# LeonhardFeiner/sparse_rcnn

Measured on AMD Instinct MI355X. Metric: active-voxels/sec fwd+bwd, ScanNet U-Net backbone, higher is better.
Workload: dtype f32

## Files before the change

sparse_rcnn_amd/csrc/scn_common.h:

```cpp
#pragma once
#include <hip/hip_runtime.h>
#include <atomic>
#include <stdint.h>
#include <stdio.h>
#include <string.h>

#include "../../include/scn_mi355x.h"

namespace scn {

extern thread_local char g_err[512];

inline int fail(int code, const char* fmt, const char* a = "", long long b = 0, long long c = 0) {
    snprintf(g_err, sizeof(g_err), fmt, a, b, c);
    return code;
}

#define SCN_HIP(expr)                                                                               \
    do {                                                                                            \
        hipError_t e_ = (expr);                                                                     \
        if (e_ != hipSuccess) {                                                                     \
            snprintf(scn::g_err, sizeof(scn::g_err), "%s failed: %s (%s:%d)", #expr,                \
                     hipGetErrorString(e_), __FILE__, __LINE__);                                    \
            return SCN_EHIP;                                                                        \
        }                                                                                           \
    } while (0)

#define SCN_LAUNCH_CHECK()                                                                          \
    do {                                                                                            \
        hipError_t e_ = hipGetLastError();                                                          \
        if (e_ != hipSuccess) {                                                                     \
            snprintf(scn::g_err, sizeof(scn::g_err), "kernel launch failed: %s (%s:%d)",            \
                     hipGetErrorString(e_), __FILE__, __LINE__);                                    \
            return SCN_EHIP;                                                                        \
        }                                                                                           \
    } while (0)

#define SCN_REQUIRE(cond)                                                                           \
    do {                                                                                            \
        if (!(cond)) {                                                                              \
            snprintf(scn::g_err, sizeof(scn::g_err), "%s: requirement failed: %s", __func__, #cond); \
            return SCN_EINVAL;                                                                      \
        }                                                                                           \
    } while (0)

enum Switch {
    SW_TS_SPLIT, SW_TS_SPLIT_MAX, SW_TS_NO_TAIL, SW_TS_W_HALF, SW_TS_W_BOTH, SW_TB_NB, SW_TB_KH, SW_TB_STREAM,
    SW_TB_NO_XORDER, SW_TS_STREAM, SW_TSS_NW, SW_EXEC_DEFER_SUMS, SW_PYRAMID_V1, SW_PYRAMID_ONE_STREAM, SW_WD_NO_T3,
    SW_WGRAD_BF16_MFMA, SW_WGRAD_SPLITS, SW_WD_NO_EVEC, SW_PYRAMID_NO_BRICKS, SW_CU_BUDGET, SW_EXP_A, SW_EXP_B, SW_TS_NO_CHAIN, SW_TS_PROG, SW_TB_NO_BINS,
    SW_EXEC_GROUP_WGRAD, SW_EXEC_GROUP_STEP, SW_COUNT
};
struct SwitchVal { bool set = false; long long i = 0; double f = 0.0; };
SwitchVal sw(Switch s);
inline int cu_budget() { const SwitchVal v = sw(SW_CU_BUDGET); return (v.set && v.i >= 32 && v.i <= 256) ? (int)v.i : 256; }

struct DeviceOnce {
    std::atomic<uint64_t> mask{0};
    static int cur() { int d = 0; return (hipGetDevice(&d) == hipSuccess && d >= 0 && d < 64) ? d : -1; }
    bool needed() const { const int d = cur(); return d < 0 || !(mask.load(std::memory_order_acquire) & (1ull << d)); }
    void done() { const int d = cur(); if (d >= 0) mask.fetch_or(1ull << d, std::memory_order_release); }
};

int wgrad_defer_group(bool on);

inline hipStream_t S(scn_stream_t s) { return reinterpret_cast<hipStream_t>(s); }

inline int64_t cdiv(int64_t a, int64_t b) { return (a + b - 1) / b; }

inline int ew_grid(int64_t work_items, int block) {
    int64_t g = cdiv(work_items, block);
    if (g > 256 * 8) g = 256 * 8;
    if (g < 1) g = 1;
    return (int)g;
}

int add_relu(const float* X, const float* X1, int64_t count, float* Y, scn_stream_t stream);
int add_relu_bf16(const uint16_t* X, const uint16_t* X1, int64_t count, uint16_t* Y, scn_stream_t stream);

}

#define SCN_EMPTY_KEY 0xFFFFFFFFFFFFFFFFull

__device__ __forceinline__ unsigned long long scn_pack_key(int x, int y, int z, int b) {
    return ((unsigned long long)(unsigned)b << 48) | ((unsigned long long)(unsigned)x << 32) |
           ((unsigned long long)(unsigned)y << 16) | (unsigned long long)(unsigned)z;
}

__device__ __forceinline__ unsigned long long scn_hash_slot(unsigned long long key, unsigned long long mask) {
    unsigned long long h = key;
    h ^= h >> 33;
    h *= 0xff51afd7ed558ccdull;
    h ^= h >> 33;
    h *= 0xc4ceb9fe1a85ec53ull;
    h ^= h >> 33;
    return h & mask;
}

__device__ __forceinline__ float scn_mask_sigmoid(float x) { return 1.f / (1.f + __expf(-x)); }

__device__ __forceinline__ float scn_box_iou(const float* as, const float* ae, float area_a, const float* bx) {
#pragma clang fp contract(off)
    float inter = 1.f;
#pragma unroll
    for (int d = 0; d < 3; ++d) {
        const float lo = fmaxf(as[d], bx[d]), hi = fminf(ae[d], bx[3 + d]);
        const float e = fmaxf((hi - lo), 0.f);
        inter = d == 0 ? e : (inter * e);
    }
    const float uni = (area_a + bx[6]) - inter;
    return (inter / uni);
}
```

sparse_rcnn_amd/csrc/scn_conv.hip:

```cpp
#include "scn_common.h"

using scn::S;
using scn::cdiv;

namespace scn {
bool gemm_lt_usable(const void* X0, const void* X1, int cx0, int cx1, const void* W);
int gemm_lt_rows(const void* X0, int cx0, const void* X1, int cx1, int64_t n, const float* W, const float* bias,
                 const void* residual, const void* relu_mask, void* Y0, int cy0, void* Y1, int cy1, int flags, bool hb,
                 scn_stream_t stream);
int gemm_lt_rules(const void* X, int cin, const int32_t* in_rows, const int32_t* out_rows, const int64_t* prefix_host,
                  int n_off, const float* W, const float* bias, const void* relu_mask, void* Y, int cout, int flags,
                  bool hb, scn_stream_t stream);
}

typedef float f32x16 __attribute__((ext_vector_type(16)));

#define MFMA(a, b, c) __builtin_amdgcn_mfma_f32_32x32x2f32((a), (b), (c), 0, 0, 0)

__device__ __forceinline__ int acc_row(int v, int h) { return (v & 3) + 8 * (v >> 2) + 4 * h; }

__device__ __forceinline__ float bf16_bits_to_f32(unsigned short h) { return __uint_as_float((unsigned)h << 16); }
__device__ __forceinline__ unsigned short f32_to_bf16_bits(float f) { return __builtin_bit_cast(unsigned short, (__bf16)f); }

template <bool FAST, bool WT, bool HB = false>
__device__ __forceinline__ void tile_mac(f32x16& acc, const float* __restrict__ xrow, bool have, int cin,
                                         const float* __restrict__ Wo, int cout, int n, bool n_ok, int h, bool relu_in) {
    const unsigned short* xh = (const unsigned short*)xrow;
    if (FAST) {
        for (int q = 0; q < cin; q += 8) {
            const int k0 = q + 4 * h;
            float4 a = make_float4(0.f, 0.f, 0.f, 0.f);
            if (HB) {
                if (have) {
                    const uint2 r = *(const uint2*)(xh + k0);
                    a = make_float4(__uint_as_float(r.x << 16), __uint_as_float(r.x & 0xffff0000u),
                                    __uint_as_float(r.y << 16), __uint_as_float(r.y & 0xffff0000u));
                }
            } else if (have) a = *(const float4*)(xrow + k0);
            if (relu_in) { a.x = fmaxf(a.x, 0.f); a.y = fmaxf(a.y, 0.f); a.z = fmaxf(a.z, 0.f); a.w = fmaxf(a.w, 0.f); }
            float4 b;
            if (WT) {
                b = n_ok ? *(const float4*)(Wo + (long long)n * cin + k0) : make_float4(0.f, 0.f, 0.f, 0.f);
            } else {
                const float* wp = Wo + (long long)k0 * cout + n;
                b.x = n_ok ? wp[0] : 0.f;
                b.y = n_ok ? wp[cout] : 0.f;
                b.z = n_ok ? wp[2 * cout] : 0.f;
                b.w = n_ok ? wp[3 * cout] : 0.f;
            }
            acc = MFMA(a.x, b.x, acc);
            acc = MFMA(a.y, b.y, acc);
            acc = MFMA(a.z, b.z, acc);
            acc = MFMA(a.w, b.w, acc);
        }
    } else {
        for (int q = 0; q < cin; q += 8) {
#pragma unroll
            for (int e = 0; e < 4; ++e) {
                const int k = q + 4 * h + e;
                const bool k_ok = k < cin;
                float a = (have && k_ok) ? (HB ? bf16_bits_to_f32(xh[k]) : xrow[k]) : 0.f;
                if (relu_in) a = fmaxf(a, 0.f);
                float b = 0.f;
                if (k_ok && n_ok) b = WT ? Wo[(long long)n * cin + k] : Wo[(long long)k * cout + n];
                acc = MFMA(a, b, acc);
            }
        }
    }
}

template <bool FAST, bool WT, bool HB = false>
__global__ __launch_bounds__(256) void k_gemm_table(const float* __restrict__ X, int cin,
                                                    const int* __restrict__ table, int n_off, long long n_out,
                                                    const float* __restrict__ W, const float* __restrict__ bias,
                                                    const float* __restrict__ residual,
                                                    const float* __restrict__ relu_mask, float* __restrict__ Y, int cout,
                                                    int flags) {
    const int lane = threadIdx.x & 63, wave = threadIdx.x >> 6;
    const int m = lane & 31, h = lane >> 5;
    const long long r0 = ((long long)blockIdx.x * 4 + wave) * 32;
    if (r0 >= n_out) return;
    const long long row = r0 + m;
    const bool row_ok = row < n_out;
    const int n0 = blockIdx.y * 32;
    const int n = n0 + m;
    const bool n_ok = n < cout;
    const bool relu_in = flags & SCN_F_RELU_IN;
    const bool rev = flags & SCN_F_OFF_REVERSE;
    const long long wstride = (long long)cin * cout;

    f32x16 acc;
#pragma unroll
    for (int v = 0; v < 16; ++v) acc[v] = 0.f;

    int idx_next = row_ok ? (table ? table[row] : (int)row) : -1;
    for (int o = 0; o < n_off; ++o) {
        const int idx = idx_next;
        if (o + 1 < n_off) idx_next = row_ok ? table[(long long)(o + 1) * n_out + row] : -1;
        if (__ballot(idx >= 0) == 0ull) continue;
        const float* Wo = W + (long long)(rev ? n_off - 1 - o : o) * wstride;
        const float* xrow = HB ? (const float*)((const unsigned short*)X + (long long)(idx >= 0 ? idx : 0) * cin)
                               : X + (long long)(idx >= 0 ? idx : 0) * cin;
        tile_mac<FAST, WT, HB>(acc, xrow, idx >= 0, cin, Wo, cout, n, n_ok, h, relu_in);
    }

    const float bv = (bias && n_ok) ? bias[n] : 0.f;
#pragma unroll
    for (int v = 0; v < 16; ++v) {
        const long long r = r0 + acc_row(v, h);
        if (r < n_out && n_ok) {
            const long long off = r * cout + n;
            float y = acc[v] + bv;
            if (HB) {
                if (residual) y += bf16_bits_to_f32(((const unsigned short*)residual)[off]);
                if (relu_mask && !(bf16_bits_to_f32(((const unsigned short*)relu_mask)[off]) > 0.f)) y = 0.f;
                ((unsigned short*)Y)[off] = f32_to_bf16_bits(y);
            } else {
                if (residual) y += residual[off];
                if (relu_mask && !(relu_mask[off] > 0.f)) y = 0.f;
                Y[off] = y;
            }
        }
    }
}

static int gemm_table_impl(const float* X, int64_t n_in, int cin, const int32_t* table, int n_off, int64_t n_out,
                           const float* W, const float* bias, const float* residual, const float* relu_mask,
                           float* Y, int cout, int flags, scn_stream_t stream, bool hb) {
    SCN_REQUIRE(n_in >= 0 && n_out >= 0 && cin >= 1 && cout >= 1 && n_off >= 1);
    SCN_REQUIRE(table || (n_off == 1 && n_in == n_out));
    if (n_out == 0) return SCN_OK;
    SCN_REQUIRE(X && W && Y);
    SCN_REQUIRE(n_out * (int64_t)cout < (1LL << 40) && cdiv(n_out, 128) < 2147483647LL);
    const bool fast = (cin % 8 == 0) && (((uintptr_t)X & 15) == 0) && (((uintptr_t)W & 15) == 0);
    const bool wt = flags & SCN_F_W_TRANSPOSED;
    if (!table && fast && !(flags & SCN_F_GEMM_V1) && n_out < 2147483647LL)
        return scn::gemm_lt_rows(X, cin, nullptr, 0, n_out, W, bias, residual, relu_mask, Y, cout, nullptr, 0, flags, hb,
                                 stream);
    dim3 grid((unsigned)cdiv(n_out, 128), (unsigned)cdiv(cout, 32));
#define LAUNCH_T(F, T, H)                                                                                     \
    hipLaunchKernelGGL((k_gemm_table<F, T, H>), grid, dim3(256), 0, S(stream), X, cin, table, n_off,          \
                       (long long)n_out, W, bias, residual, relu_mask, Y, cout, flags)
#define PICK_T(H)                                                                                             \
    do {                                                                                                      \
        if (fast && wt) LAUNCH_T(true, true, H);                                                              \
        else if (fast) LAUNCH_T(true, false, H);                                                              \
        else if (wt) LAUNCH_T(false, true, H);                                                                \
        else LAUNCH_T(false, false, H);                                                                       \
    } while (0)
    if (hb) PICK_T(true); else PICK_T(false);
#undef PICK_T
#undef LAUNCH_T
    SCN_LAUNCH_CHECK();
    return SCN_OK;
}

extern "C" int scn_gemm_table(const float* X, int64_t n_in, int cin, const int32_t* table, int n_off, int64_t n_out,
                              const float* W, const float* bias, const float* residual, const float* relu_mask,
                              float* Y, int cout, int flags, scn_stream_t stream) {
    return gemm_table_impl(X, n_in, cin, table, n_off, n_out, W, bias, residual, relu_mask, Y, cout, flags, stream, false);
}

extern "C" int scn_gemm_table_bf16(const uint16_t* X, int64_t n_in, int cin, const int32_t* table, int n_off,
                                   int64_t n_out, const float* W, const float* bias, const uint16_t* residual,
                                   const uint16_t* relu_mask, uint16_t* Y, int cout, int flags, scn_stream_t stream) {
    return gemm_table_impl((const float*)X, n_in, cin, table, n_off, n_out, W, bias, (const float*)residual,
                           (const float*)relu_mask, (float*)Y, cout, flags, stream, true);
}

struct SegTiles {
    long long rule_start[33];
    long long tile_start[33];
    int n_off;
};

template <bool FAST, bool WT, bool HB = false>
__global__ __launch_bounds__(256) void k_gemm_rules(const float* __restrict__ X, int cin,
                                                    const int* __restrict__ in_rows, const int* __restrict__ out_rows,
                                                    SegTiles seg, const float* __restrict__ W,
                                                    const float* __restrict__ bias, const float* __restrict__ relu_mask,
                                                    float* __restrict__ Y, int cout, int flags) {
    const int lane = threadIdx.x & 63, wave = threadIdx.x >> 6;
    const int m = lane & 31, h = lane >> 5;
    const long long tile = (long long)blockIdx.x * 4 + wave;
    if (tile >= seg.tile_start[seg.n_off]) return;
    int o = 0;
    while (tile >= seg.tile_start[o + 1]) ++o;
    const long long p0 = seg.rule_start[o] + (tile - seg.tile_start[o]) * 32;
    const long long p_end = seg.rule_start[o + 1];
    const long long p = p0 + m;
    const bool p_ok = p < p_end;
    const int idx = p_ok ? in_rows[p] : -1;
    const int orow = p_ok ? out_rows[p] : -1;
    const int n0 = blockIdx.y * 32;
    const int n = n0 + m;
    const bool n_ok = n < cout;

    f32x16 acc;
#pragma unroll
    for (int v = 0; v < 16; ++v) acc[v] = 0.f;
    const float* Wo = W + (long long)o * cin * cout;
    const float* xrow = HB ? (const float*)((const unsigned short*)X + (long long)(idx >= 0 ? idx : 0) * cin)
                           : X + (long long)(idx >= 0 ? idx : 0) * cin;
    tile_mac<FAST, WT, HB>(acc, xrow, idx >= 0, cin, Wo, cout, n, n_ok, h, flags & SCN_F_RELU_IN);

    const float bv = (bias && n_ok) ? bias[n] : 0.f;
#pragma unroll
    for (int v = 0; v < 16; ++v) {
        const int r = __shfl(orow, acc_row(v, h));
        if (r >= 0 && n_ok) {
            const long long off = (long long)r * cout + n;
            float y = acc[v] + bv;
            if (HB) {
                if (relu_mask && !(bf16_bits_to_f32(((const unsigned short*)relu_mask)[off]) > 0.f)) y = 0.f;
                ((unsigned short*)Y)[off] = f32_to_bf16_bits(y);
            } else {
                if (relu_mask && !(relu_mask[off] > 0.f)) y = 0.f;
                Y[off] = y;
            }
        }
    }
}

static int make_seg_tiles(const int64_t* prefix_host, int n_off, int tile, SegTiles& seg) {
    seg.n_off = n_off;
    seg.rule_start[0] = prefix_host[0];
    seg.tile_start[0] = 0;
    for (int o = 0; o < n_off; ++o) {
        int64_t cnt = prefix_host[o + 1] - prefix_host[o];
        if (cnt < 0) return SCN_EINVAL;
        seg.rule_start[o + 1] = prefix_host[o + 1];
        seg.tile_start[o + 1] = seg.tile_start[o] + cdiv(cnt, tile);
    }
    return SCN_OK;
}

static int gemm_rules_impl(const float* X, int cin, const int32_t* in_rows, const int32_t* out_rows,
                           const int64_t* prefix_host, int n_off, const float* W, const float* bias,
                           const float* relu_mask, float* Y, int cout, int flags, scn_stream_t stream, bool hb) {
    SCN_REQUIRE(prefix_host && n_off >= 1 && n_off <= 32 && cin >= 1 && cout >= 1);
    SegTiles seg;
    SCN_REQUIRE(make_seg_tiles(prefix_host, n_off, 32, seg) == SCN_OK);
    const long long tiles = seg.tile_start[n_off];
    if (tiles == 0) return SCN_OK;
    SCN_REQUIRE(X && in_rows && out_rows && W && Y);
    const bool fast = (cin % 8 == 0) && (((uintptr_t)X & 15) == 0) && (((uintptr_t)W & 15) == 0);
    const bool wt = flags & SCN_F_W_TRANSPOSED;
    if (fast && cout > 32 && !(flags & SCN_F_GEMM_V1))
        return scn::gemm_lt_rules(X, cin, in_rows, out_rows, prefix_host, n_off, W, bias, relu_mask, Y, cout, flags, hb,
                                  stream);
    dim3 grid((unsigned)cdiv(tiles, 4), (unsigned)cdiv(cout, 32));
#define LAUNCH_R(F, T, H)                                                                                     \
    hipLaunchKernelGGL((k_gemm_rules<F, T, H>), grid, dim3(256), 0, S(stream), X, cin, in_rows, out_rows, seg, \
                       W, bias, relu_mask, Y, cout, flags)
#define PICK_R(H)                                                                                             \
    do {                                                                                                      \
        if (fast && wt) LAUNCH_R(true, true, H);                                                              \
        else if (fast) LAUNCH_R(true, false, H);                                                              \
        else if (wt) LAUNCH_R(false, true, H);                                                                \
        else LAUNCH_R(false, false, H);                                                                       \
    } while (0)
    if (hb) PICK_R(true); else PICK_R(false);
#undef PICK_R
#undef LAUNCH_R
    SCN_LAUNCH_CHECK();
    return SCN_OK;
}

extern "C" int scn_gemm_rules(const float* X, int cin, const int32_t* in_rows, const int32_t* out_rows,
                              const int64_t* prefix_host, int n_off, const float* W, const float* bias,
                              const float* relu_mask, float* Y, int cout, int flags, scn_stream_t stream) {
    return gemm_rules_impl(X, cin, in_rows, out_rows, prefix_host, n_off, W, bias, relu_mask, Y, cout, flags, stream,
                           false);
}

extern "C" int scn_gemm_rules_bf16(const uint16_t* X, int cin, const int32_t* in_rows, const int32_t* out_rows,
                                   const int64_t* prefix_host, int n_off, const float* W, const float* bias,
                                   const uint16_t* relu_mask, uint16_t* Y, int cout, int flags, scn_stream_t stream) {
    return gemm_rules_impl((const float*)X, cin, in_rows, out_rows, prefix_host, n_off, W, bias,
                           (const float*)relu_mask, (float*)Y, cout, flags, stream, true);
}

template <bool HB>
__global__ __launch_bounds__(256) void k_colsum_partial(const float* __restrict__ dY, long long n, int c,
                                                        float* __restrict__ partial) {
    const unsigned short* dYh = (const unsigned short*)dY;
    const long long rows_per_block = (n + gridDim.x - 1) / gridDim.x;
    const long long r_lo = blockIdx.x * rows_per_block;
    long long r_hi = r_lo + rows_per_block;
    if (r_hi > n) r_hi = n;
    __shared__ float red[256];
    for (int c0 = 0; c0 < c; c0 += 256) {
        const int width = min(256, c - c0);
        const int lanes_per_row = width;
        const int rows_par = 256 / lanes_per_row > 0 ? 256 / lanes_per_row : 1;
        const int col = threadIdx.x % lanes_per_row;
        const int rsub = threadIdx.x / lanes_per_row;
        float s = 0.f;
        if (rsub < rows_par)
            for (long long r = r_lo + rsub; r < r_hi; r += rows_par)
                s += HB ? bf16_bits_to_f32(dYh[r * c + c0 + col]) : dY[r * c + c0 + col];
        red[threadIdx.x] = (rsub < rows_par) ? s : 0.f;
        __syncthreads();
        if (threadIdx.x < width) {
            float t = 0.f;
            for (int k = 0; k < rows_par; ++k) t += red[k * lanes_per_row + threadIdx.x];
            partial[(long long)blockIdx.x * c + c0 + threadIdx.x] = t;
        }
        __syncthreads();
    }
}

__global__ __launch_bounds__(256) void k_colsum_final(const float* __restrict__ partial, int nblk, int c,
                                                      float* __restrict__ db) {
    const int col = blockIdx.x;
    float s = 0.f;
    for (int b = threadIdx.x; b < nblk; b += 256) s += partial[(long long)b * c + col];
#pragma unroll
    for (int d = 32; d >= 1; d >>= 1) s += __shfl_down(s, d);
    __shared__ float w[4];
    if ((threadIdx.x & 63) == 0) w[threadIdx.x >> 6] = s;
    __syncthreads();
    if (threadIdx.x == 0) db[col] = (w[0] + w[1]) + (w[2] + w[3]);
}

static int colsum_impl(const float* dY, int64_t n, int c, float* db, void* scratch, scn_stream_t stream, bool hb) {
    SCN_REQUIRE(n >= 0 && c >= 1 && db && scratch);
    int nblk = (int)(n < SCN_COLSUM_BLOCKS * 8 ? cdiv(n, 8) : SCN_COLSUM_BLOCKS);
    if (nblk < 1) nblk = 1;
    if (n > 0) SCN_REQUIRE(dY);
    if (hb)
        hipLaunchKernelGGL(k_colsum_partial<true>, dim3(nblk), dim3(256), 0, S(stream), dY, (long long)n, c, (float*)scratch);
    else
        hipLaunchKernelGGL(k_colsum_partial<false>, dim3(nblk), dim3(256), 0, S(stream), dY, (long long)n, c, (float*)scratch);
    SCN_LAUNCH_CHECK();
    hipLaunchKernelGGL(k_colsum_final, dim3(c), dim3(256), 0, S(stream), (const float*)scratch, nblk, c, db);
    SCN_LAUNCH_CHECK();
    return SCN_OK;
}

extern "C" int scn_colsum(const float* dY, int64_t n, int c, float* db, void* scratch, scn_stream_t stream) {
    return colsum_impl(dY, n, c, db, scratch, stream, false);
}

extern "C" int scn_colsum_bf16(const uint16_t* dY, int64_t n, int c, float* db, void* scratch, scn_stream_t stream) {
    return colsum_impl((const float*)dY, n, c, db, scratch, stream, true);
}
```

sparse_rcnn_amd/csrc/scn_debug.hip:

```cpp
#include <stdlib.h>

#include <mutex>

#include "scn_common.h"

namespace scn {
namespace {
struct Entry { const char* name; SwitchVal v; };
Entry g_sw[SW_COUNT] = {
    {"SCN_TS_SPLIT", {}},        {"SCN_TS_SPLIT_MAX", {}},  {"SCN_TS_NO_TAIL", {}},       {"SCN_TS_W_HALF", {}},
    {"SCN_TS_W_BOTH", {}},       {"SCN_TB_NB", {}},         {"SCN_TB_KH", {}},            {"SCN_TB_STREAM", {}},
    {"SCN_TB_NO_XORDER", {}},    {"SCN_TS_STREAM", {}},     {"SCN_TSS_NW", {}},           {"SCN_EXEC_DEFER_SUMS", {}},
    {"SCN_PYRAMID_V1", {}},      {"SCN_PYRAMID_ONE_STREAM", {}}, {"SCN_WD_NO_T3", {}},    {"SCN_WGRAD_BF16_MFMA", {}},
    {"SCN_WGRAD_SPLITS", {}},    {"SCN_WD_NO_EVEC", {}},    {"SCN_PYRAMID_NO_BRICKS", {}},            {"SCN_CU_BUDGET", {}},
    {"SCN_EXP_A", {}},           {"SCN_EXP_B", {}},         {"SCN_TS_NO_CHAIN", {}},
    {"SCN_TS_PROG", {}},         {"SCN_TB_NO_BINS", {}},    {"SCN_EXEC_GROUP_WGRAD", {}},
    {"SCN_EXEC_GROUP_STEP", {}},
};
std::once_flag g_once;
std::mutex g_mu;

void assign(SwitchVal& v, const char* s) {
    v.set = s != nullptr;
    v.i = s ? atoll(s) : 0;
    v.f = s ? atof(s) : 0.0;
}
void load_env() {
    for (int k = 0; k < SW_COUNT; ++k) assign(g_sw[k].v, getenv(g_sw[k].name));
}
}

SwitchVal sw(Switch s) {
    std::call_once(g_once, load_env);
    std::lock_guard<std::mutex> lock(g_mu);
    return g_sw[s].v;
}
}

extern "C" int scn_debug_set(const char* name, const char* value) {
    SCN_REQUIRE(name != nullptr);
    std::call_once(scn::g_once, scn::load_env);
    std::lock_guard<std::mutex> lock(scn::g_mu);
    for (int k = 0; k < scn::SW_COUNT; ++k)
        if (strcmp(scn::g_sw[k].name, name) == 0) {
            scn::assign(scn::g_sw[k].v, value);
            return SCN_OK;
        }
    return scn::fail(SCN_EINVAL, "scn_debug_set: no switch named %s", name);
}

extern "C" int scn_debug_get(const char* name, int* is_set, int64_t* value) {
    SCN_REQUIRE(name != nullptr);
    for (int k = 0; k < scn::SW_COUNT; ++k)
        if (strcmp(scn::g_sw[k].name, name) == 0) {
            const scn::SwitchVal v = scn::sw((scn::Switch)k);
            if (is_set) *is_set = v.set ? 1 : 0;
            if (value) *value = v.i;
            return SCN_OK;
        }
    return scn::fail(SCN_EINVAL, "scn_debug_get: no switch named %s", name);
}
```

sparse_rcnn_amd/csrc/scn_gemm_lt.hip:

```cpp
#include "scn_common.h"

using scn::S;
using scn::cdiv;

typedef float f32x16 __attribute__((ext_vector_type(16)));
#define MFMA32(a, b, c) __builtin_amdgcn_mfma_f32_32x32x2f32((a), (b), (c), 0, 0, 0)

namespace {

constexpr int KC = 32;
constexpr int PITCH = KC + 4;

struct LtSeg {
    long long rule_start[33];
    long long tile_start[33];
    int n_off;
};

struct LtArgs {
    const void* X0; const void* X1; int cx0, cx1;
    void* Y0; void* Y1; int cy0, cy1;
    const float* W; const float* bias; const void* residual; const void* relu_mask;
    const int* in_rows; const int* out_rows;
    long long n;
    int cin, cout, flags;
};

__device__ __forceinline__ float bf16w(unsigned short h) { return __uint_as_float((unsigned)h << 16); }
__device__ __forceinline__ unsigned short bf16n(float f) { return __builtin_bit_cast(unsigned short, (__bf16)f); }
__device__ __forceinline__ int acc_row(int v, int h) { return (v & 3) + 8 * (v >> 2) + 4 * h; }

template <int NC, bool WT, bool HB, bool RULES>
__global__ __launch_bounds__(256) void k_gemm_lt(LtArgs a, LtSeg seg) {
    constexpr int RT = 128 / NC;
    constexpr int NP = RT / 32;
    __shared__ float As[2][RT * PITCH];
    const int tid = threadIdx.x, lane = tid & 63, wave = tid >> 6;
    const int m = lane & 31, h = lane >> 5;
    const int rsub = wave / NC, cchunk = wave % NC;

    long long p0, p_end;
    const float* Wo = a.W;
    if (RULES) {
        const long long tile = blockIdx.x;
        int o = 0;
        while (tile >= seg.tile_start[o + 1]) ++o;
        p0 = seg.rule_start[o] + (tile - seg.tile_start[o]) * RT;
        p_end = seg.rule_start[o + 1];
        Wo += (long long)o * a.cin * a.cout;
    } else {
        p0 = (long long)blockIdx.x * RT;
        p_end = a.n;
    }
    const int n = blockIdx.y * (NC * 32) + cchunk * 32 + m;
    const bool n_ok = n < a.cout;
    const bool relu_in = a.flags & SCN_F_RELU_IN;

    int srow[NP];
#pragma unroll
    for (int i = 0; i < NP; ++i) {
        const long long p = p0 + (tid + 256 * i) / 8;
        srow[i] = -1;
        if (p < p_end) srow[i] = RULES ? a.in_rows[p] : (int)p;
    }
    const int c4 = 4 * (tid & 7);

    auto load_a = [&](int kc, float4 (&st)[NP]) {
        const int k = kc + c4;
        const bool second = a.cx1 && k >= a.cx0;
        const char* base = (const char*)(second ? a.X1 : a.X0);
        const int pitch = second ? a.cx1 : a.cx0, kk = second ? k - a.cx0 : k;
#pragma unroll
        for (int i = 0; i < NP; ++i) {
            float4 v = make_float4(0.f, 0.f, 0.f, 0.f);
            if (srow[i] >= 0 && k < a.cin) {
                if (HB) {
                    const uint2 r = *(const uint2*)(base + 2 * ((long long)srow[i] * pitch + kk));
                    v = make_float4(__uint_as_float(r.x << 16), __uint_as_float(r.x & 0xffff0000u),
                                    __uint_as_float(r.y << 16), __uint_as_float(r.y & 0xffff0000u));
                } else {
                    v = *(const float4*)(base + 4 * ((long long)srow[i] * pitch + kk));
                }
                if (relu_in) { v.x = fmaxf(v.x, 0.f); v.y = fmaxf(v.y, 0.f); v.z = fmaxf(v.z, 0.f); v.w = fmaxf(v.w, 0.f); }
            }
            st[i] = v;
        }
    };
    auto park_a = [&](int buf, const float4 (&st)[NP]) {
#pragma unroll
        for (int i = 0; i < NP; ++i) *(float4*)&As[buf][((tid + 256 * i) / 8) * PITCH + c4] = st[i];
    };
    auto load_b = [&](int kc, float4 (&b)[4]) {
#pragma unroll
        for (int q = 0; q < 4; ++q) {
            const int k0 = kc + 8 * q + 4 * h;
            float4 v = make_float4(0.f, 0.f, 0.f, 0.f);
            if (n_ok && k0 < a.cin) {
                if (WT) {
                    v = *(const float4*)(Wo + (long long)n * a.cin + k0);
                } else {
                    const float* wp = Wo + (long long)k0 * a.cout + n;
                    v = make_float4(wp[0], wp[a.cout], wp[2 * a.cout], wp[3 * a.cout]);
                }
            }
            b[q] = v;
        }
    };

    f32x16 acc;
#pragma unroll
    for (int v = 0; v < 16; ++v) acc[v] = 0.f;

    float4 st[NP], bcur[4], bnext[4];
    load_a(0, st);
    load_b(0, bcur);
    park_a(0, st);
    __syncthreads();
    const int n_chunks = (a.cin + KC - 1) / KC;
    for (int c = 0; c < n_chunks; ++c) {
        const int buf = c & 1;
        const bool more = c + 1 < n_chunks;
        if (more) {
            load_a((c + 1) * KC, st);
            load_b((c + 1) * KC, bnext);
        }
        const float* arow = &As[buf][(rsub * 32 + m) * PITCH + 4 * h];
#pragma unroll
        for (int q = 0; q < 4; ++q) {
            const float4 av = *(const float4*)(arow + 8 * q);
            acc = MFMA32(av.x, bcur[q].x, acc);
            acc = MFMA32(av.y, bcur[q].y, acc);
            acc = MFMA32(av.z, bcur[q].z, acc);
            acc = MFMA32(av.w, bcur[q].w, acc);
        }
        if (more) {
            park_a(buf ^ 1, st);
#pragma unroll
            for (int q = 0; q < 4; ++q) bcur[q] = bnext[q];
        }
        __syncthreads();
    }

    const long long prow = p0 + rsub * 32 + m;
    long long orow_l = -1;
    if (prow < p_end) orow_l = RULES ? (long long)a.out_rows[prow] : prow;
    const int orow_i = (int)orow_l;
    const float bv = (a.bias && n_ok) ? a.bias[n] : 0.f;
    const bool second = a.cy1 && n >= a.cy0;
    char* ybase = (char*)(second ? a.Y1 : a.Y0);
    const int ypitch = second ? a.cy1 : a.cy0, yn = second ? n - a.cy0 : n;
#pragma unroll
    for (int v = 0; v < 16; ++v) {
        const int r = __shfl(orow_i, acc_row(v, h));
        if (r >= 0 && n_ok) {
            const long long off = (long long)r * ypitch + yn;
            float y = acc[v] + bv;
            if (HB) {
                if (a.residual) y += bf16w(((const unsigned short*)a.residual)[off]);
                if (a.relu_mask && !(bf16w(((const unsigned short*)a.relu_mask)[off]) > 0.f)) y = 0.f;
                ((unsigned short*)ybase)[off] = bf16n(y);
            } else {
                if (a.residual) y += ((const float*)a.residual)[off];
                if (a.relu_mask && !(((const float*)a.relu_mask)[off] > 0.f)) y = 0.f;
                ((float*)ybase)[off] = y;
            }
        }
    }
}

template <bool WT, bool HB, bool RULES>
int launch_nc(const LtArgs& a, const LtSeg& seg, long long tiles_of_128, scn_stream_t stream) {
    const int nc = a.cout <= 32 ? 1 : a.cout <= 64 ? 2 : 4;
    const unsigned gy = (unsigned)cdiv(a.cout, nc * 32);
    (void)tiles_of_128;
    long long gx;
    if (RULES) gx = seg.tile_start[seg.n_off];
    else gx = cdiv(a.n, 128 / nc);
    if (gx <= 0) return SCN_OK;
    SCN_REQUIRE(gx < 2147483647LL);
    dim3 grid((unsigned)gx, gy);
    if (nc == 1) hipLaunchKernelGGL((k_gemm_lt<1, WT, HB, RULES>), grid, dim3(256), 0, S(stream), a, seg);
    else if (nc == 2) hipLaunchKernelGGL((k_gemm_lt<2, WT, HB, RULES>), grid, dim3(256), 0, S(stream), a, seg);
    else hipLaunchKernelGGL((k_gemm_lt<4, WT, HB, RULES>), grid, dim3(256), 0, S(stream), a, seg);
    SCN_LAUNCH_CHECK();
    return SCN_OK;
}

template <bool RULES>
int launch_lt(const LtArgs& a, const LtSeg& seg, bool hb, scn_stream_t stream) {
    const bool wt = a.flags & SCN_F_W_TRANSPOSED;
    if (hb) return wt ? launch_nc<true, true, RULES>(a, seg, 0, stream) : launch_nc<false, true, RULES>(a, seg, 0, stream);
    return wt ? launch_nc<true, false, RULES>(a, seg, 0, stream) : launch_nc<false, false, RULES>(a, seg, 0, stream);
}

}

namespace scn {

bool gemm_lt_usable(const void* X0, const void* X1, int cx0, int cx1, const void* W) {
    auto al = [](const void* p) { return ((uintptr_t)p & 15) == 0; };
    return cx0 % 8 == 0 && cx1 % 8 == 0 && al(X0) && al(X1) && al(W);
}

int gemm_lt_rows(const void* X0, int cx0, const void* X1, int cx1, int64_t n, const float* W, const float* bias,
                 const void* residual, const void* relu_mask, void* Y0, int cy0, void* Y1, int cy1, int flags, bool hb,
                 scn_stream_t stream) {
    LtArgs a{};
    a.X0 = X0; a.X1 = X1; a.cx0 = cx0; a.cx1 = cx1;
    a.Y0 = Y0; a.Y1 = Y1; a.cy0 = cy0; a.cy1 = cy1;
    a.W = W; a.bias = bias; a.residual = residual; a.relu_mask = relu_mask;
    a.n = n; a.cin = cx0 + cx1; a.cout = cy0 + cy1; a.flags = flags;
    LtSeg seg{};
    return launch_lt<false>(a, seg, hb, stream);
}

int gemm_lt_rules(const void* X, int cin, const int32_t* in_rows, const int32_t* out_rows, const int64_t* prefix_host,
                  int n_off, const float* W, const float* bias, const void* relu_mask, void* Y, int cout, int flags,
                  bool hb, scn_stream_t stream) {
    LtArgs a{};
    a.X0 = X; a.cx0 = cin; a.Y0 = Y; a.cy0 = cout;
    a.W = W; a.bias = bias; a.relu_mask = relu_mask; a.in_rows = in_rows; a.out_rows = out_rows;
    a.cin = cin; a.cout = cout; a.flags = flags;
    const int nc = cout <= 32 ? 1 : cout <= 64 ? 2 : 4;
    const int rt = 128 / nc;
    LtSeg seg{};
    seg.n_off = n_off;
    seg.rule_start[0] = prefix_host[0];
    seg.tile_start[0] = 0;
    for (int o = 0; o < n_off; ++o) {
        const int64_t cnt = prefix_host[o + 1] - prefix_host[o];
        SCN_REQUIRE(cnt >= 0);
        seg.rule_start[o + 1] = prefix_host[o + 1];
        seg.tile_start[o + 1] = seg.tile_start[o] + cdiv(cnt, rt);
    }
    return launch_lt<true>(a, seg, hb, stream);
}

}

extern "C" int scn_gemm_rows2(const void* X0, int cx0, const void* X1, int cx1, int64_t n, const float* W,
                              const float* bias, const void* residual, const void* relu_mask, void* Y0, int cy0, void* Y1,
                              int cy1, int flags, int bf16_storage, scn_stream_t stream) {
    SCN_REQUIRE(n >= 0 && cx0 >= 8 && cx1 >= 0 && cy0 >= 1 && cy1 >= 0);
    SCN_REQUIRE(cx0 % 8 == 0 && cx1 % 8 == 0);
    SCN_REQUIRE((cx1 == 0) == (X1 == nullptr) && (cy1 == 0) == (Y1 == nullptr));
    SCN_REQUIRE(!(cx1 && cy1));
    SCN_REQUIRE(cy1 == 0 || (!residual && !relu_mask));
    SCN_REQUIRE(n < 2147483647LL);
    if (n == 0) return SCN_OK;
    SCN_REQUIRE(X0 && W && Y0);
    SCN_REQUIRE(scn::gemm_lt_usable(X0, X1, cx0, cx1, W));
    return scn::gemm_lt_rows(X0, cx0, X1, cx1, n, W, bias, residual, relu_mask, Y0, cy0, Y1, cy1, flags,
                             bf16_storage != 0, stream);
}
```

Measured before the change: 28.52 million.

## Make LT GEMM persistent with deep A prefetch and early epilogue loads

Reworks the MFMA row/rule GEMM kernel into a grid-sized launch. Blocks loop over flattened (row-tile, column-block) tiles and prefetch the next tile's rows and first chunk. For larger cin it adds a variant that keeps several K-chunks of A in flight, using unconditional clamped loads plus masks. It also issues residual/relu-mask loads before the final MAC, and uses readfirstlane scalar offsets and 32-bit addressing. The aim is to hide global-load latency and cut launch and tail cost, at the price of higher register pressure (launch_bounds 256,4), an occupancy query, and more complex control flow.

After: 28.52 million. No clear change (-0.0%).

```diff
diff --git a/sparse_rcnn_amd/csrc/scn_common.h b/sparse_rcnn_amd/csrc/scn_common.h
--- a/sparse_rcnn_amd/csrc/scn_common.h
+++ b/sparse_rcnn_amd/csrc/scn_common.h
@@ -48,7 +48,7 @@
     SW_TS_SPLIT, SW_TS_SPLIT_MAX, SW_TS_NO_TAIL, SW_TS_W_HALF, SW_TS_W_BOTH, SW_TB_NB, SW_TB_KH, SW_TB_STREAM,
     SW_TB_NO_XORDER, SW_TS_STREAM, SW_TSS_NW, SW_EXEC_DEFER_SUMS, SW_PYRAMID_V1, SW_PYRAMID_ONE_STREAM, SW_WD_NO_T3,
     SW_WGRAD_BF16_MFMA, SW_WGRAD_SPLITS, SW_WD_NO_EVEC, SW_PYRAMID_NO_BRICKS, SW_CU_BUDGET, SW_EXP_A, SW_EXP_B, SW_TS_NO_CHAIN, SW_TS_PROG, SW_TB_NO_BINS,
-    SW_EXEC_GROUP_WGRAD, SW_EXEC_GROUP_STEP, SW_COUNT
+    SW_EXEC_GROUP_WGRAD, SW_EXEC_GROUP_STEP, SW_GEMM_LT_WG, SW_COUNT
 };
 struct SwitchVal { bool set = false; long long i = 0; double f = 0.0; };
 SwitchVal sw(Switch s);
diff --git a/sparse_rcnn_amd/csrc/scn_conv.hip b/sparse_rcnn_amd/csrc/scn_conv.hip
--- a/sparse_rcnn_amd/csrc/scn_conv.hip
+++ b/sparse_rcnn_amd/csrc/scn_conv.hip
@@ -4,7 +4,7 @@
 using scn::cdiv;
 
 namespace scn {
-bool gemm_lt_usable(const void* X0, const void* X1, int cx0, int cx1, const void* W);
+bool gemm_lt_usable(const void* X0, const void* X1, int cx0, int cx1, const void* W, int cout);
 int gemm_lt_rows(const void* X0, int cx0, const void* X1, int cx1, int64_t n, const float* W, const float* bias,
                  const void* residual, const void* relu_mask, void* Y0, int cy0, void* Y1, int cy1, int flags, bool hb,
                  scn_stream_t stream);
@@ -134,7 +134,8 @@
     SCN_REQUIRE(n_out * (int64_t)cout < (1LL << 40) && cdiv(n_out, 128) < 2147483647LL);
     const bool fast = (cin % 8 == 0) && (((uintptr_t)X & 15) == 0) && (((uintptr_t)W & 15) == 0);
     const bool wt = flags & SCN_F_W_TRANSPOSED;
-    if (!table && fast && !(flags & SCN_F_GEMM_V1) && n_out < 2147483647LL)
+    if (!table && fast && scn::gemm_lt_usable(X, nullptr, cin, 0, W, cout) && !(flags & SCN_F_GEMM_V1) &&
+        n_out < 2147483647LL)
         return scn::gemm_lt_rows(X, cin, nullptr, 0, n_out, W, bias, residual, relu_mask, Y, cout, nullptr, 0, flags, hb,
                                  stream);
     dim3 grid((unsigned)cdiv(n_out, 128), (unsigned)cdiv(cout, 32));
@@ -246,7 +247,7 @@
     SCN_REQUIRE(X && in_rows && out_rows && W && Y);
     const bool fast = (cin % 8 == 0) && (((uintptr_t)X & 15) == 0) && (((uintptr_t)W & 15) == 0);
     const bool wt = flags & SCN_F_W_TRANSPOSED;
-    if (fast && cout > 32 && !(flags & SCN_F_GEMM_V1))
+    if (fast && cout > 32 && scn::gemm_lt_usable(X, nullptr, cin, 0, W, cout) && !(flags & SCN_F_GEMM_V1))
         return scn::gemm_lt_rules(X, cin, in_rows, out_rows, prefix_host, n_off, W, bias, relu_mask, Y, cout, flags, hb,
                                   stream);
     dim3 grid((unsigned)cdiv(tiles, 4), (unsigned)cdiv(cout, 32));
diff --git a/sparse_rcnn_amd/csrc/scn_debug.hip b/sparse_rcnn_amd/csrc/scn_debug.hip
--- a/sparse_rcnn_amd/csrc/scn_debug.hip
+++ b/sparse_rcnn_amd/csrc/scn_debug.hip
@@ -15,7 +15,7 @@
     {"SCN_WGRAD_SPLITS", {}},    {"SCN_WD_NO_EVEC", {}},    {"SCN_PYRAMID_NO_BRICKS", {}},            {"SCN_CU_BUDGET", {}},
     {"SCN_EXP_A", {}},           {"SCN_EXP_B", {}},         {"SCN_TS_NO_CHAIN", {}},
     {"SCN_TS_PROG", {}},         {"SCN_TB_NO_BINS", {}},    {"SCN_EXEC_GROUP_WGRAD", {}},
-    {"SCN_EXEC_GROUP_STEP", {}},
+    {"SCN_EXEC_GROUP_STEP", {}}, {"SCN_GEMM_LT_WG", {}},
 };
 std::once_flag g_once;
 std::mutex g_mu;
diff --git a/sparse_rcnn_amd/csrc/scn_gemm_lt.hip b/sparse_rcnn_amd/csrc/scn_gemm_lt.hip
--- a/sparse_rcnn_amd/csrc/scn_gemm_lt.hip
+++ b/sparse_rcnn_amd/csrc/scn_gemm_lt.hip
@@ -8,6 +8,12 @@
 
 namespace {
 
+#ifndef LT_EARLY
+#define LT_EARLY 1
+#endif
+#ifndef LT_DEEP
+#define LT_DEEP 4
+#endif
 constexpr int KC = 32;
 constexpr int PITCH = KC + 4;
 
@@ -24,182 +30,374 @@
     const int* in_rows; const int* out_rows;
     long long n;
     int cin, cout, flags;
+    long long n_tiles; int gy;
 };
 
 __device__ __forceinline__ float bf16w(unsigned short h) { return __uint_as_float((unsigned)h << 16); }
 __device__ __forceinline__ unsigned short bf16n(float f) { return __builtin_bit_cast(unsigned short, (__bf16)f); }
 __device__ __forceinline__ int acc_row(int v, int h) { return (v & 3) + 8 * (v >> 2) + 4 * h; }
 
-template <int NC, bool WT, bool HB, bool RULES>
-__global__ __launch_bounds__(256) void k_gemm_lt(LtArgs a, LtSeg seg) {
+struct LtTile {
+    long long p0, p_end;
+    const float* Wo;
+    int cb;
+};
+
+template <int NC, bool WT, bool HB, bool RULES, int AD>
+__global__ __launch_bounds__(256, 4) void k_gemm_lt(LtArgs a, LtSeg seg) {
     constexpr int RT = 128 / NC;
     constexpr int NP = RT / 32;
+    constexpr int ES = HB ? 2 : 4;
+    constexpr bool EARLY = LT_EARLY && WT && NC > 1;
     __shared__ float As[2][RT * PITCH];
-    const int tid = threadIdx.x, lane = tid & 63, wave = tid >> 6;
+    const int tid = threadIdx.x, lane = tid & 63, wave = __builtin_amdgcn_readfirstlane(tid >> 6);
     const int m = lane & 31, h = lane >> 5;
     const int rsub = wave / NC, cchunk = wave % NC;
-
-    long long p0, p_end;
-    const float* Wo = a.W;
-    if (RULES) {
-        const long long tile = blockIdx.x;
-        int o = 0;
-        while (tile >= seg.tile_start[o + 1]) ++o;
-        p0 = seg.rule_start[o] + (tile - seg.tile_start[o]) * RT;
-        p_end = seg.rule_start[o + 1];
-        Wo += (long long)o * a.cin * a.cout;
-    } else {
-        p0 = (long long)blockIdx.x * RT;
-        p_end = a.n;
-    }
-    const int n = blockIdx.y * (NC * 32) + cchunk * 32 + m;
-    const bool n_ok = n < a.cout;
     const bool relu_in = a.flags & SCN_F_RELU_IN;
-
-    int srow[NP];
-#pragma unroll
-    for (int i = 0; i < NP; ++i) {
-        const long long p = p0 + (tid + 256 * i) / 8;
-        srow[i] = -1;
-        if (p < p_end) srow[i] = RULES ? a.in_rows[p] : (int)p;
-    }
-    const int c4 = 4 * (tid & 7);
-
-    auto load_a = [&](int kc, float4 (&st)[NP]) {
+    const int c4 = 4 * (tid & 7), srl = tid >> 3;
+
+    auto tile_of = [&](long long t, int& o, LtTile& T) {
+        const long long rt = a.gy == 1 ? t : t / a.gy;
+        T.cb = (int)(t - rt * a.gy);
+        if (RULES) {
+            while (rt >= seg.tile_start[o + 1]) ++o;
+            T.p0 = seg.rule_start[o] + (rt - seg.tile_start[o]) * RT;
+            T.p_end = seg.rule_start[o + 1];
+            T.Wo = a.W + (long long)o * a.cin * a.cout;
+        } else {
+            T.p0 = rt * RT;
+            T.p_end = a.n;
+            T.Wo = a.W;
+        }
+    };
+    auto stage_rows = [&](const LtTile& T, int (&sr)[NP]) {
+        if (!RULES) return;
+#pragma unroll
+        for (int i = 0; i < NP; ++i) {
+            const long long p = T.p0 + srl + 32 * i;
+            const bool ok = p < T.p_end;
+            const int v = a.in_rows[ok ? p : T.p_end - 1];
+            sr[i] = ok ? v : -1;
+        }
+    };
+    auto out_row = [&](const LtTile& T) -> int {
+        if (!RULES) return -1;
+        const long long p = T.p0 + rsub * 32 + m;
+        const bool ok = p < T.p_end;
+        const int v = a.out_rows[ok ? p : T.p_end - 1];
+        return ok ? v : -1;
+    };
+    auto load_a = [&](const LtTile& T, const int (&sr)[NP], int kc, float4 (&st)[NP]) {
         const int k = kc + c4;
         const bool second = a.cx1 && k >= a.cx0;
         const char* base = (const char*)(second ? a.X1 : a.X0);
         const int pitch = second ? a.cx1 : a.cx0, kk = second ? k - a.cx0 : k;
+        const char* tbase = base + ES * (T.p0 * pitch);
 #pragma unroll
         for (int i = 0; i < NP; ++i) {
             float4 v = make_float4(0.f, 0.f, 0.f, 0.f);
-            if (srow[i] >= 0 && k < a.cin) {
+            const bool ok = RULES ? sr[i] >= 0 : T.p0 + srl + 32 * i < T.p_end;
+            if (ok && k < a.cin) {
+                const char* src = RULES ? base + ES * ((long long)sr[i] * pitch + kk)
+                                        : tbase + (unsigned)(ES * ((srl + 32 * i) * pitch + kk));
                 if (HB) {
-                    const uint2 r = *(const uint2*)(base + 2 * ((long long)srow[i] * pitch + kk));
+                    const uint2 r = *(const uint2*)src;
                     v = make_float4(__uint_as_float(r.x << 16), __uint_as_float(r.x & 0xffff0000u),
                                     __uint_as_float(r.y << 16), __uint_as_float(r.y & 0xffff0000u));
                 } else {
-                    v = *(const float4*)(base + 4 * ((long long)srow[i] * pitch + kk));
+                    v = *(const float4*)src;
                 }
-                if (relu_in) { v.x = fmaxf(v.x, 0.f); v.y = fmaxf(v.y, 0.f); v.z = fmaxf(v.z, 0.f); v.w = fmaxf(v.w, 0.f); }
             }
             st[i] = v;
         }
     };
-    auto park_a = [&](int buf, const float4 (&st)[NP]) {
-#pragma unroll
-        for (int i = 0; i < NP; ++i) *(float4*)&As[buf][((tid + 256 * i) / 8) * PITCH + c4] = st[i];
-    };
-    auto load_b = [&](int kc, float4 (&b)[4]) {
+    auto park_a = [&](int buf, const float4 (&st)[NP], int okm) {
+#pragma unroll
+        for (int i = 0; i < NP; ++i) {
+            float4 v = st[i];
+            if (!((okm >> i) & 1)) v = make_float4(0.f, 0.f, 0.f, 0.f);
+            if (relu_in) { v.x = fmaxf(v.x, 0.f); v.y = fmaxf(v.y, 0.f); v.z = fmaxf(v.z, 0.f); v.w = fmaxf(v.w, 0.f); }
+            *(float4*)&As[buf][(srl + 32 * i) * PITCH + c4] = v;
+        }
+    };
+    auto load_b = [&](const LtTile& T, int kc, float4 (&b)[4]) {
+        const int n = T.cb * (NC * 32) + cchunk * 32 + m;
 #pragma unroll
         for (int q = 0; q < 4; ++q) {
             const int k0 = kc + 8 * q + 4 * h;
             float4 v = make_float4(0.f, 0.f, 0.f, 0.f);
-            if (n_ok && k0 < a.cin) {
+            if (n < a.cout && k0 < a.cin) {
                 if (WT) {
-                    v = *(const float4*)(Wo + (long long)n * a.cin + k0);
+                    v = *(const float4*)(T.Wo + (unsigned)(n * a.cin + k0));
                 } else {
-                    const float* wp = Wo + (long long)k0 * a.cout + n;
-                    v = make_float4(wp[0], wp[a.cout], wp[2 * a.cout], wp[3 * a.cout]);
+                    const unsigned wl = (unsigned)(4 * h * a.cout + n);
+                    float e[4];
+#pragma unroll
+                    for (int j = 0; j < 4; ++j) {
+                        const unsigned ws = __builtin_amdgcn_readfirstlane((unsigned)((kc + 8 * q + j) * a.cout));
+                        e[j] = T.Wo[ws + wl];
+                    }
+                    v = make_float4(e[0], e[1], e[2], e[3]);
                 }
             }
             b[q] = v;
         }
     };
 
-    f32x16 acc;
-#pragma unroll
-    for (int v = 0; v < 16; ++v) acc[v] = 0.f;
-
-    float4 st[NP], bcur[4], bnext[4];
-    load_a(0, st);
-    load_b(0, bcur);
-    park_a(0, st);
+    auto load_a_u = [&](const LtTile& T, const int (&sr)[NP], int kc, float4 (&st)[NP], int& okm) {
+        okm = 0;
+        const int k = kc + c4, kq = k < a.cin ? k : a.cin - 4;
+        const bool second = a.cx1 && kq >= a.cx0;
+        const char* base = (const char*)(second ? a.X1 : a.X0);
+        const int pitch = second ? a.cx1 : a.cx0, kk = second ? kq - a.cx0 : kq;
+        const char* tbase = base + ES * (T.p0 * pitch);
+        const int last_row = (int)(T.p_end - 1 - T.p0 < RT - 1 ? T.p_end - 1 - T.p0 : RT - 1);
+#pragma unroll
+        for (int i = 0; i < NP; ++i) {
+            const int lr = srl + 32 * i;
+            const bool ok = (RULES ? sr[i] >= 0 : lr <= last_row) && k < a.cin;
+            const char* src = RULES ? base + ES * ((long long)(sr[i] > 0 ? sr[i] : 0) * pitch + kk)
+                                    : tbase + (unsigned)(ES * ((lr < last_row ? lr : last_row) * pitch + kk));
+            float4 v;
+            if (HB) {
+                const uint2 r = *(const uint2*)src;
+                v = make_float4(__uint_as_float(r.x << 16), __uint_as_float(r.x & 0xffff0000u),
+                                __uint_as_float(r.y << 16), __uint_as_float(r.y & 0xffff0000u));
+            } else {
+                v = *(const float4*)src;
+            }
+            okm |= (ok ? 1 : 0) << i;
+            st[i] = v;
+        }
+    };
+    auto load_b_u = [&](const LtTile& T, int kc, float4 (&b)[4]) {
+        const int n = T.cb * (NC * 32) + cchunk * 32 + m, nq = n < a.cout ? n : a.cout - 1;
+#pragma unroll
+        for (int q = 0; q < 4; ++q) {
+            const int k0 = kc + 8 * q + 4 * h, kq = k0 < a.cin ? k0 : a.cin - 4;
+            float4 v;
+            if (WT) {
+                v = *(const float4*)(T.Wo + (unsigned)(nq * a.cin + kq));
+            } else {
+                const unsigned w0 = (unsigned)(kq * a.cout + nq), wc = (unsigned)a.cout;
+                v = make_float4(T.Wo[w0], T.Wo[w0 + wc], T.Wo[w0 + 2 * wc], T.Wo[w0 + 3 * wc]);
+            }
+            b[q] = v;
+        }
+    };
+
+    const int n_chunks = (a.cin + KC - 1) / KC;
+    const long long G = gridDim.x;
+    long long t = blockIdx.x;
+    int o = 0, o_n = 0;
+    LtTile T, Tn;
+    tile_of(t, o, T);
+    Tn = T;
+    int srow[NP], srow_n[NP];
+#pragma unroll
+    for (int i = 0; i < NP; ++i) srow[i] = srow_n[i] = -1;
+    stage_rows(T, srow);
+
+    int orow = out_row(T), orow_n = -1;
+
+    static_assert(AD == 1 || AD % 2 == 0, "the B fragments of chunk c wait in slot c % 2");
+    float4 st[NP], bq[2][4];
+    float4 (&bcur)[4] = bq[0], (&bnext)[4] = bq[1];
+    float4 sq[AD][NP];
+    int okq[AD];
+    auto chunk_at = [&](int c) { return (c < n_chunks ? c : n_chunks - 1) * KC; };
+    if (AD == 1) {
+        load_a(T, srow, 0, st);
+        load_b(T, 0, bcur);
+        park_a(0, st, -1);
+    } else {
+#pragma unroll
+        for (int j = 0; j < AD; ++j) load_a_u(T, srow, chunk_at(j), sq[j], okq[j]);
+        load_b_u(T, 0, bcur);
+        park_a(0, sq[0], okq[0]);
+    }
     __syncthreads();
-    const int n_chunks = (a.cin + KC - 1) / KC;
-    for (int c = 0; c < n_chunks; ++c) {
-        const int buf = c & 1;
-        const bool more = c + 1 < n_chunks;
-        if (more) {
-            load_a((c + 1) * KC, st);
-            load_b((c + 1) * KC, bnext);
-        }
-        const float* arow = &As[buf][(rsub * 32 + m) * PITCH + 4 * h];
-#pragma unroll
-        for (int q = 0; q < 4; ++q) {
-            const float4 av = *(const float4*)(arow + 8 * q);
-            acc = MFMA32(av.x, bcur[q].x, acc);
-            acc = MFMA32(av.y, bcur[q].y, acc);
-            acc = MFMA32(av.z, bcur[q].z, acc);
-            acc = MFMA32(av.w, bcur[q].w, acc);
-        }
-        if (more) {
-            park_a(buf ^ 1, st);
+    int buf = 0;
+    for (;;) {
+        const long long t_n = t + G;
+        const bool have_next = AD == 1 && t_n < a.n_tiles;
+        if (have_next) {
+            o_n = o;
+            tile_of(t_n, o_n, Tn);
+            stage_rows(Tn, srow_n);
+            orow_n = out_row(Tn);
+        }
+        f32x16 acc;
+#pragma unroll
+        for (int v = 0; v < 16; ++v) acc[v] = 0.f;
+
+        auto mac_chunk = [&](const float4 (&b)[4], int kc) {
+            const float* arow = &As[buf][(rsub * 32 + m) * PITCH + 4 * h];
+#pragma unroll
+            for (int q = 0; q < 4; ++q) {
+                const float4 av = *(const float4*)(arow + 8 * q);
+                float4 bv = b[q];
+                if (AD > 1 && !(kc + 8 * q + 4 * h < a.cin)) bv = make_float4(0.f, 0.f, 0.f, 0.f);
+                acc = MFMA32(av.x, bv.x, acc);
+                acc = MFMA32(av.y, bv.y, acc);
+                acc = MFMA32(av.z, bv.z, acc);
+                acc = MFMA32(av.w, bv.w, acc);
+            }
+        };
+        auto advance = [&]() {
+            park_a(buf ^ 1, st, -1);
 #pragma unroll
             for (int q = 0; q < 4; ++q) bcur[q] = bnext[q];
-        }
+        };
+        if (AD > 1) {
+            for (int c0 = 0; c0 + 1 < n_chunks; c0 += AD) {
+#pragma unroll
+                for (int j = 0; j < AD; ++j) {
+                    const int c = c0 + j;
+                    if (c + 1 >= n_chunks) break;
+                    load_a_u(T, srow, chunk_at(c + AD), sq[j], okq[j]);
+                    load_b_u(T, (c + 1) * KC, bq[(j + 1) & 1]);
+                    mac_chunk(bq[j & 1], c * KC);
+                    park_a(buf ^ 1, sq[(j + 1) % AD], okq[(j + 1) % AD]);
+                    __syncthreads();
+                    buf ^= 1;
+                }
+            }
+        }
+        for (int c = 0; AD == 1 && c + 1 < n_chunks; ++c) {
+            load_a(T, srow, (c + 1) * KC, st);
+            load_b(T, (c + 1) * KC, bnext);
+            mac_chunk(bcur, c * KC);
+            advance();
+            __syncthreads();
+            buf ^= 1;
+        }
+        if (have_next) {
+            load_a(Tn, srow_n, 0, st);
+            load_b(Tn, 0, bnext);
+        }
+
+        const int n = T.cb * (NC * 32) + cchunk * 32 + m;
+        const bool n_ok = n < a.cout;
+        const bool second = a.cy1 && n >= a.cy0;
+        const int ypitch = second ? a.cy1 : a.cy0, yn = n_ok ? (second ? n - a.cy0 : n) : 0;
+        const long long r0 = T.p0 + rsub * 32;
+        const long long r0c = r0 < T.p_end ? r0 : T.p_end - 1;
+        const int rows_here = (int)(T.p_end - r0 < 32 ? T.p_end - r0 : 32);
+        auto row_of = [&](int v) { return RULES ? __shfl(orow, acc_row(v, h)) : (acc_row(v, h) < rows_here ? 0 : -1); };
+        auto elem = [&](const void* base, int v, int r, bool clamp) -> const char* {
+            if (RULES) {
+                return (const char*)base + ES * ((long long)(r > 0 ? r : 0) * ypitch + yn);
+            }
+            int lr = acc_row(v, h);
+            if (clamp) lr = lr < rows_here ? lr : (rows_here > 0 ? rows_here - 1 : 0);
+            return (const char*)base + ES * ((clamp ? r0c : r0) * ypitch) + (unsigned)(ES * (lr * ypitch + yn));
+        };
+        auto value = [&](const char* p) { return HB ? bf16w(*(const unsigned short*)p) : *(const float*)p; };
+
+        const void* early = a.residual ? a.residual : a.relu_mask;
+        float epi[16], bv = 0.f;
+        if (a.bias) bv = a.bias[n_ok ? n : 0];
+        if (EARLY && early) {
+#pragma unroll
+            for (int v = 0; v < 16; ++v) epi[v] = value(elem(early, v, row_of(v), true));
+        }
+        if (AD > 1 && ((n_chunks - 1) & 1)) mac_chunk(bq[1], (n_chunks - 1) * KC);
+        else mac_chunk(bq[0], (n_chunks - 1) * KC);
+        if (have_next) advance();
         __syncthreads();
-    }
-
-    const long long prow = p0 + rsub * 32 + m;
-    long long orow_l = -1;
-    if (prow < p_end) orow_l = RULES ? (long long)a.out_rows[prow] : prow;
-    const int orow_i = (int)orow_l;
-    const float bv = (a.bias && n_ok) ? a.bias[n] : 0.f;
-    const bool second = a.cy1 && n >= a.cy0;
-    char* ybase = (char*)(second ? a.Y1 : a.Y0);
-    const int ypitch = second ? a.cy1 : a.cy0, yn = second ? n - a.cy0 : n;
-#pragma unroll
-    for (int v = 0; v < 16; ++v) {
-        const int r = __shfl(orow_i, acc_row(v, h));
-        if (r >= 0 && n_ok) {
-            const long long off = (long long)r * ypitch + yn;
-            float y = acc[v] + bv;
-            if (HB) {
-                if (a.residual) y += bf16w(((const unsigned short*)a.residual)[off]);
-                if (a.relu_mask && !(bf16w(((const unsigned short*)a.relu_mask)[off]) > 0.f)) y = 0.f;
-                ((unsigned short*)ybase)[off] = bf16n(y);
-            } else {
-                if (a.residual) y += ((const float*)a.residual)[off];
-                if (a.relu_mask && !(((const float*)a.relu_mask)[off] > 0.f)) y = 0.f;
-                ((float*)ybase)[off] = y;
-            }
-        }
-    }
-}
-
-template <bool WT, bool HB, bool RULES>
-int launch_nc(const LtArgs& a, const LtSeg& seg, long long tiles_of_128, scn_stream_t stream) {
-    const int nc = a.cout <= 32 ? 1 : a.cout <= 64 ? 2 : 4;
-    const unsigned gy = (unsigned)cdiv(a.cout, nc * 32);
-    (void)tiles_of_128;
-    long long gx;
-    if (RULES) gx = seg.tile_start[seg.n_off];
-    else gx = cdiv(a.n, 128 / nc);
-    if (gx <= 0) return SCN_OK;
-    SCN_REQUIRE(gx < 2147483647LL);
-    dim3 grid((unsigned)gx, gy);
-    if (nc == 1) hipLaunchKernelGGL((k_gemm_lt<1, WT, HB, RULES>), grid, dim3(256), 0, S(stream), a, seg);
-    else if (nc == 2) hipLaunchKernelGGL((k_gemm_lt<2, WT, HB, RULES>), grid, dim3(256), 0, S(stream), a, seg);
-    else hipLaunchKernelGGL((k_gemm_lt<4, WT, HB, RULES>), grid, dim3(256), 0, S(stream), a, seg);
+        buf ^= 1;
+
+        if (!n_ok) bv = 0.f;
+        char* ybase = (char*)(second ? a.Y1 : a.Y0);
+#pragma unroll
+        for (int v = 0; v < 16; ++v) {
+            const int r = row_of(v);
+            if (r >= 0 && n_ok) {
+                float y = acc[v] + bv;
+                if (EARLY) {
+                    if (a.residual) {
+                        y += epi[v];
+                        if (a.relu_mask && !(value(elem(a.relu_mask, v, r, false)) > 0.f)) y = 0.f;
+                    } else if (a.relu_mask && !(epi[v] > 0.f)) {
+                        y = 0.f;
+                    }
+                } else {
+                    if (a.residual) y += value(elem(a.residual, v, r, false));
+                    if (a.relu_mask && !(value(elem(a.relu_mask, v, r, false)) > 0.f)) y = 0.f;
+                }
+                char* dst = const_cast<char*>(elem(ybase, v, r, false));
+                if (HB) *(unsigned short*)dst = bf16n(y);
+                else *(float*)dst = y;
+            }
+        }
+        if (!have_next) break;
+        t = t_n; o = o_n; T = Tn; orow = orow_n;
+#pragma unroll
+        for (int i = 0; i < NP; ++i) srow[i] = srow_n[i];
+    }
+}
+
+template <int NC, bool WT, bool HB, bool RULES, int AD>
+int launch_k(LtArgs& a, const LtSeg& seg, scn_stream_t stream, bool* fits) {
+    static std::atomic<int> per_cu{0};
+    int occ = per_cu.load(std::memory_order_relaxed);
+    if (occ == 0) {
+        SCN_HIP(hipOccupancyMaxActiveBlocksPerMultiprocessor(&occ, k_gemm_lt<NC, WT, HB, RULES, AD>, 256, 0));
+        if (occ < 1) occ = 1;
+        per_cu.store(occ, std::memory_order_relaxed);
+    }
+    const long long slots = (long long)scn::cu_budget() * occ;
+    long long g = cdiv(a.n_tiles, cdiv(a.n_tiles, slots));
+    const scn::SwitchVal cap = scn::sw(scn::SW_GEMM_LT_WG);
+    if (AD > 1) {
+        *fits = a.n_tiles <= slots && !(cap.set && cap.i >= 1);
+        if (!*fits) return SCN_OK;
+        g = a.n_tiles;
+    } else if (cap.set && cap.i >= 1) {
+        g = a.n_tiles < cap.i ? a.n_tiles : cap.i;
+    }
+    SCN_REQUIRE(g >= 1 && g < 2147483647LL);
+    hipLaunchKernelGGL((k_gemm_lt<NC, WT, HB, RULES, AD>), dim3((unsigned)g), dim3(256), 0, S(stream), a, seg);
     SCN_LAUNCH_CHECK();
     return SCN_OK;
+}
+
+template <bool WT, bool HB, bool RULES>
+int launch_nc(LtArgs a, const LtSeg& seg, scn_stream_t stream) {
+    const int nc = a.cout <= 32 ? 1 : a.cout <= 64 ? 2 : 4;
+    a.gy = (int)cdiv(a.cout, nc * 32);
+    const long long row_tiles = RULES ? seg.tile_start[seg.n_off] : cdiv(a.n, 128 / nc);
+    if (row_tiles <= 0) return SCN_OK;
+    SCN_REQUIRE(row_tiles < 2147483647LL / a.gy);
+    a.n_tiles = row_tiles * a.gy;
+    bool fits = false;
+    if (nc > 1 && a.cin > 2 * KC) {
+        const int rc = nc == 2 ? launch_k<2, WT, HB, RULES, LT_DEEP>(a, seg, stream, &fits)
+                               : launch_k<4, WT, HB, RULES, LT_DEEP>(a, seg, stream, &fits);
+        if (rc != SCN_OK || fits) return rc;
+    }
+    if (nc == 1) return launch_k<1, WT, HB, RULES, 1>(a, seg, stream, &fits);
+    if (nc == 2) return launch_k<2, WT, HB, RULES, 1>(a, seg, stream, &fits);
+    return launch_k<4, WT, HB, RULES, 1>(a, seg, stream, &fits);
 }
 
 template <bool RULES>
 int launch_lt(const LtArgs& a, const LtSeg& seg, bool hb, scn_stream_t stream) {
     const bool wt = a.flags & SCN_F_W_TRANSPOSED;
-    if (hb) return wt ? launch_nc<true, true, RULES>(a, seg, 0, stream) : launch_nc<false, true, RULES>(a, seg, 0, stream);
-    return wt ? launch_nc<true, false, RULES>(a, seg, 0, stream) : launch_nc<false, false, RULES>(a, seg, 0, stream);
+    if (hb) return wt ? launch_nc<true, true, RULES>(a, seg, stream) : launch_nc<false, true, RULES>(a, seg, stream);
+    return wt ? launch_nc<true, false, RULES>(a, seg, stream) : launch_nc<false, false, RULES>(a, seg, stream);
 }
 
 }
 
 namespace scn {
 
-bool gemm_lt_usable(const void* X0, const void* X1, int cx0, int cx1, const void* W) {
+bool gemm_lt_usable(const void* X0, const void* X1, int cx0, int cx1, const void* W, int cout) {
     auto al = [](const void* p) { return ((uintptr_t)p & 15) == 0; };
-    return cx0 % 8 == 0 && cx1 % 8 == 0 && al(X0) && al(X1) && al(W);
+    const int64_t cin = (int64_t)cx0 + cx1;
+    return cx0 % 8 == 0 && cx1 % 8 == 0 && al(X0) && al(X1) && al(W) && cin <= (1 << 20) && cout <= (1 << 20) &&
+           cin * cout < (1LL << 30);
 }
 
 int gemm_lt_rows(const void* X0, int cx0, const void* X1, int cx1, int64_t n, const float* W, const float* bias,
@@ -249,7 +447,7 @@
     SCN_REQUIRE(n < 2147483647LL);
     if (n == 0) return SCN_OK;
     SCN_REQUIRE(X0 && W && Y0);
-    SCN_REQUIRE(scn::gemm_lt_usable(X0, X1, cx0, cx1, W));
+    SCN_REQUIRE(scn::gemm_lt_usable(X0, X1, cx0, cx1, W, cy0 + cy1));
     return scn::gemm_lt_rows(X0, cx0, X1, cx1, n, W, bias, residual, relu_mask, Y0, cy0, Y1, cy1, flags,
                              bf16_storage != 0, stream);
 }
```
